# jsourati/nn-active-learning

Hardware: AMD Instinct MI355X
Metric: patches/sec Fisher-scored (32^3, 2-class) (higher is better)
Workload: dtype f32 (fp32 operands split into 16-bit pieces on the 16-bit MFMA, fp32 accumulate: fp16 pairs - 22-23 bits kept per operand, three products - in the conv under the head (forward + backward), in dec1's forward launch and in the other backward launches; bf16 triples - all 24 bits, exact, six products -

## Files before the change

include/alq.h:

```cpp
#ifndef ALQ_H
#define ALQ_H

#include <stddef.h>
#include <stdint.h>

#ifdef __cplusplus
extern "C" {
#endif

typedef struct alq_ctx alq_ctx;
typedef struct alq_model alq_model;

enum { ALQ_OK = 0, ALQ_EINVAL = -1, ALQ_EHIP = -2, ALQ_ENOMEM = -3, ALQ_EUNSUPPORTED = -4 };

enum { ALQ_CONV = 0, ALQ_CONVT = 1, ALQ_POOL = 2, ALQ_FC = 3 };

typedef struct {
    int32_t type;
    int32_t cout;
    int32_t k[3];
    int32_t s[3];
    int32_t relu;
    int32_t skip_src;
} alq_layer_t;
// ... 240 lines not shown
                         int64_t *elems_out);

int alq_debug_set_stamp_buffer(void *d_buf);
int alq_debug_set(int key, int value);
enum {
    ALQ_INFO_SUBNORMALS_OK = 0,
    ALQ_INFO_C3D_FWD = 1,
    ALQ_INFO_C3D_BWD = 2,
    ALQ_INFO_C3D_ONE_ACC = 3,
    ALQ_INFO_FLIP_OVERFLOW = 5,
    ALQ_INFO_F16_DERIVED = 6,
    ALQ_INFO_T3D_FWD = 7,
    ALQ_INFO_T3D_BWD = 8,
    ALQ_INFO_E3D_BWD = 9,
    ALQ_INFO_D3D_FWD = 10,
    ALQ_INFO_D3D_BWD = 11,
    ALQ_INFO_F3D_FWD = 12,
    ALQ_INFO_C3D_BWD_FORM = 13,
    ALQ_INFO_HOST_PACK_ELEMS = 14,
    ALQ_INFO_LSUM = 15,
    ALQ_INFO_DCP_FORM = 16,
    ALQ_INFO_E3D_BWD_FORM = 17,
    ALQ_INFO_C3D_BWD_WAVES = 19,
    ALQ_INFO_C3D_BWD_GRID = 20
};
int alq_model_engine_info(alq_model *m, int what);

int alq_synth_patches(alq_ctx *ctx, uint64_t seed, int64_t first_id, int64_t n,
                      int64_t elems_per_patch, float *d_out);

enum { ALQ_SRC_F32 = 0, ALQ_SRC_F64 = 1, ALQ_SRC_I16 = 2, ALQ_SRC_U8 = 3 };
int alq_vol_pack(alq_ctx *ctx, const void *const *d_src, int m, int src_type, const int32_t *dims, float *d_out);
int alq_mask_pack(alq_ctx *ctx, const uint8_t *d_src, const int32_t *dims, uint8_t *d_out);
int alq_slice_batch_check(const int32_t *h_dims, int nvol, const int32_t *h_desc, int b, const int32_t *crop, int C);
int alq_slice_batch(alq_ctx *ctx, const float *const *h_vols, const uint8_t *const *h_masks, const int32_t *h_dims, int nvol, int m,
                    const int32_t *h_desc, int b, const int32_t *crop, int C, float *d_X, int32_t *d_lab, int64_t *d_counts);
int64_t alq_slice_batch_trip_rows(void);
int alq_slice_batch_launch_samples(void);

#ifdef __cplusplus
}
#endif
#endif
```

nn-active-learning_amd/csrc/alq_internal.h:

```cpp
#pragma once
#include <hip/hip_runtime.h>

#include <cstdint>
#include <cstdio>
#include <memory>
#include <string>
#include <vector>

#include "alq.h"
#include "engine_switches.h"
#include "model_plan.h"

namespace alq {

#define ALQ_HIP(expr)                                                                     \
    do {                                                                                  \
        hipError_t e_ = (expr);                                                           \
        if (e_ != hipSuccess) {                                                           \
            ::alq::set_error("%s:%d: %s -> %s", __FILE__, __LINE__, #expr,               \
                             hipGetErrorString(e_));                                      \
            return ALQ_EHIP;                                                              \
        }                                                                                 \
    } while (0)

// ... 323 lines not shown
void c3d_fwd_pack(C3dPlan *plan, const std::vector<float> &Bmat );
int c3d_fwd_launch(alq_ctx *ctx, const C3dPlan &plan, const View &in, const float *bias, int N, const unsigned *amaxA, const unsigned *amaxB,
                   const float *fc_W, float *fc_part, float *asum_part, unsigned char *fc_bits, float flip_tau);
int c3d_bwd_build(const View &fwd_in, const View &fwd_out, const int k[3], const int lo[3], const int s[3], C3dPlan *plan);
void c3d_bwd_pack(C3dPlan *plan, const std::vector<float> &Bmat_fwd );
void c3d_presplit_vec(const float *v, long long F, int e, std::vector<unsigned short> *out);
int c3d_bwd_launch(alq_ctx *ctx, const C3dPlan &plan, int N, const unsigned char *bits, const void *vec16, int e_in, const unsigned char *maskA,
                   float *dB, float *sumA, float *sumB, int rows_per_wave = 8, int waves_per_simd = 1 ,
                   int *grid_out = nullptr );

struct T3dPlan {
    bool ok = false;
    int kind = 0;
    int w_exp = 0;
    double flops_per_patch = 0;
    std::vector<unsigned short> h_W;
    void *d_W = nullptr;
};
int t3d_build(const View &in, const View &out, const int k[3], const int lo[3], const int s[3], T3dPlan *fwd, T3dPlan *bwd);
void t3d_fwd_pack(T3dPlan *plan, const float *W );
void t3d_bwd_pack(T3dPlan *plan, const float *W);
void t3d8_fwd_pack(T3dPlan *plan, const float *W );
void t3d8_bwd_pack(T3dPlan *plan, const float *W );
int t3d8_bwd_launch(alq_ctx *ctx, const T3dPlan &plan, const View &dout, const View &din, int N, float in_bound, const unsigned char *mask_bits, float *dsum);
int t3d_fwd_launch(alq_ctx *ctx, const T3dPlan &plan, const View &in, const View &out, const float *bias, int N, float *osum, unsigned *out_amax);
int t3d_bwd_launch(alq_ctx *ctx, const T3dPlan &plan, const View &dout, const View &din, int N, float in_bound, const unsigned char *mask_bits,
                   float *dsum);

struct E3dPlan {
    bool ok = false;
    int w_exp = 0;
    double flops_per_patch = 0;
    std::vector<unsigned short> h_Whi, h_Wlo;
    void *d_Whi = nullptr, *d_Wlo = nullptr;
};
int e3d_build(const View &in, const View &out, const int k[3], const int lo[3], const int s[3], E3dPlan *plan);
void e3d_pack(E3dPlan *plan, const float *W );
int e3d_bwd_launch(alq_ctx *ctx, const E3dPlan &plan, int N, const float *skip, const float *dpool, const unsigned char *am2, const unsigned char *sg2,
                   const unsigned char *am1, const unsigned char *sg1, float *dsum2, float *dsum1, float in_bound,
                   bool rows );

struct D3dPlan {
    bool ok = false;
    int w_exp = 0;
    double flops_per_patch = 0;
    std::vector<unsigned short> h_Whi, h_Wlo;
    void *d_Whi = nullptr, *d_Wlo = nullptr;
    std::vector<unsigned short> h_Bhi, h_Blo;
    void *d_Bhi = nullptr, *d_Blo = nullptr;
};
// ... 257 lines not shown
```

nn-active-learning_amd/csrc/engine_switches.h:

```cpp
#ifndef ALQ_ENGINE_SWITCHES_H
#define ALQ_ENGINE_SWITCHES_H
#include <cstddef>
#include <cstdlib>

namespace alq {

enum Knob {
    KNOB_REPEAT = 0,
    KNOB_FLAGS = 1,
    KNOB_NO_BWD_FUSE = 2,
    KNOB_NO_FWD_FUSE = 3,
    KNOB_NO_V3 = 4,
    KNOB_NO_V4 = 5,
    KNOB_NO_POOL_FIRST = 6,
    KNOB_NO_CONV_POOL = 7,
    KNOB_DCP_NARROW = 8,
    KNOB_E3D_GRID_CAP = 9,
    KNOB_C3B7_GRID_CAP = 10,
    ALQ_NKNOBS = 11
};

struct EngineSwitches {
    int knobs[ALQ_NKNOBS] = {0, 0, 0, 0, 0, 0, 0, 0, 0, 0, 0};
    int disable_v2 = 0;
    int disable_v3 = 0;
    int disable_v4 = 0;
    int no_fcgemm = 0;
    int no_split = 0;
    int no_wide2d_rule = 0;
    int no_v3_f16 = 0;
    int no_v3_f16_fwd = 0;
    int no_co_split = 0;
    int no_co_split_f16 = 0;
    int no_class_tiles = 0;
    int no_fc_bits = 0;
    int no_fc_fuse = 0;
    int no_fc_f16 = 0;
    int no_fc_f16_fwd = 0;
    int f16_derived_mask = 0;
    int has_f16_derived_mask = 0;
    int no_f16x2 = 0;
    int no_xcd_order = 0;
    int no_fixed = 0;
    int no_bound16 = 0;
    int no_flipfix = 0;
    int no_presplit = 0;
    int no_signs = 0;
    int no_signs0 = 0;
    int f16_fwd_mask = -1;
    int no_f16_derived = 0;
    int no_light_kernels = 0;
    int no_c3d = 0;
    int c3_bwd_rows = 7;
    int c3_bwd_waves = 2;
    int no_e3d = 0;
    int e3d_rows = 0;
    int no_d3d = 0;
    int no_d3b = 0;
    int no_f3d = 0;
    int no_t3d = 0;
};

enum SwitchRule {
    SW_PRESENT,
    SW_FIRST_IS_1,
    SW_ATOI_EQ,
    SW_INT,
    SW_ROWS
};

struct SwitchRow {
    const char *env;
    size_t member;
    SwitchRule rule;
    int arg;
};

#define ALQ_SW(env, member, rule, arg) {env, offsetof(EngineSwitches, member), rule, arg}
inline const SwitchRow kSwitchTable[] = {
// ... 46 lines not shown
    ALQ_SW("ALQ_NO_T3D", no_t3d, SW_PRESENT, 0),
};
#undef ALQ_SW
inline const int kNumSwitchRows = (int)(sizeof(kSwitchTable) / sizeof(kSwitchTable[0]));

inline int &switch_member(EngineSwitches &sw, const SwitchRow &row) {
    return *reinterpret_cast<int *>(reinterpret_cast<char *>(&sw) + row.member);
}

inline EngineSwitches read_engine_switches() {
    EngineSwitches sw;
    for (const SwitchRow &row : kSwitchTable) {
        const char *v = std::getenv(row.env);
        int &dst = switch_member(sw, row);
        switch (row.rule) {
            case SW_PRESENT:    if (v) dst = 1; break;
            case SW_FIRST_IS_1: if (v && v[0] == '1') dst = 1; break;
            case SW_ATOI_EQ:    if (v && std::atoi(v) == row.arg) dst = 1; break;
            case SW_INT:        if (v) dst = std::atoi(v); break;
            case SW_ROWS:       dst = (v && std::atoi(v) == 4) ? 4 : ((v && std::atoi(v) == 8) ? 8 : 7); break;
        }
    }
    if (const char *v = std::getenv("ALQ_C3D_BWD_WAVES")) sw.c3_bwd_waves = std::atoi(v) == 1 ? 1 : 2;
    return sw;
}

}
#endif
```

nn-active-learning_amd/csrc/igemm2.hip:

```cpp
#include "alq_internal.h"

#include <algorithm>
#include <cmath>
#include <cstring>

namespace alq {

typedef float f32x4 __attribute__((ext_vector_type(4)));
typedef float f32x2 __attribute__((ext_vector_type(2)));

#ifdef ALQ_STAMPS
#define STAMP(var) asm volatile("s_memtime %0\n\ts_waitcnt lgkmcnt(0)" : "=s"(var)::"memory")
#define PHASE_END(idx)                         \
    do {                                       \
        unsigned long long t_now_;             \
        STAMP(t_now_);                         \
        ph[idx] += t_now_ - t_last;            \
        t_last = t_now_;                       \
    } while (0)
#else
#define PHASE_END(idx) do {} while (0)
#endif

constexpr int I2_CBP = 12;
// ... 461 lines not shown
}

void igemm2_pack_weights(Igemm2Plan *p2, const std::vector<float> &Bmat) {
    const Igemm2Args &a = p2->a;
    const int NTW = p2->NTW, Ci = a.Ci, Co = a.Co;
    p2->h_W.assign((size_t)a.nchunks * a.ntaps * NTW * 128, 0.f);
    for (int ch = 0; ch < a.nchunks; ++ch)
        for (int tp = 0; tp < a.ntaps; ++tp)
            for (int nt = 0; nt < NTW; ++nt)
                for (int lane = 0; lane < 64; ++lane)
                    for (int s = 0; s < 2; ++s) {
                        const int c = ch * 8 + 2 * (lane >> 4) + s;
                        const int co = nt * 16 + (lane & 15);
                        if (co < Co)
                            p2->h_W[((((size_t)ch * a.ntaps + tp) * NTW + nt) * 64 + lane) * 2 + s] =
                                Bmat[((size_t)tp * Ci + c) * Co + co];
                    }
}

unsigned long long *g_igemm2_dbg = nullptr;
int g_no_f16x2 = 0;
int g_no_xcd_order = 0;
int g_no_fixed = 0;
int g_dbg_knobs[ALQ_NKNOBS] = {0, 0, 0, 0, 0, 0, 0, 0, 0, 0, 0};

template <int NTW, bool WRES, int GEO, bool SUMS>
static int launch2_s(alq_ctx *ctx, const Igemm2Plan &plan, const Igemm2Args &a, unsigned grid) {
    auto kfn = igemm2_kernel<NTW, WRES, GEO, SUMS>;
    if (plan.lds_bytes > 64 * 1024)
        ALQ_HIP(hipFuncSetAttribute(reinterpret_cast<const void *>(kfn), hipFuncAttributeMaxDynamicSharedMemorySize,
                                    (int)plan.lds_bytes));
    hipLaunchKernelGGL(kfn, dim3(grid), dim3(256), plan.lds_bytes, ctx->stream, a);
    ALQ_HIP(hipGetLastError());
    return ALQ_OK;
}

template <int NTW, bool WRES, int GEO>
static int launch2_t(alq_ctx *ctx, const Igemm2Plan &plan, const Igemm2Args &a, unsigned grid) {
    return (a.osumA || a.osumB) ? launch2_s<NTW, WRES, GEO, true>(ctx, plan, a, grid)
                                : launch2_s<NTW, WRES, GEO, false>(ctx, plan, a, grid);
}

int igemm2_launch(alq_ctx *ctx, const Igemm2Plan &plan, const View &in, const View &out, const float *bias, int relu,
                  int accumulate, int N, int prof_cls, const Igemm2Fuse *fuse) {
    Igemm2Args a = plan.a;
    ALQ_REQUIRE(in.C == a.Ci && in.D == a.ID && in.H == a.IH && in.W == a.IW, ALQ_EINVAL,
                "igemm2: input view does not match plan");
// ... 53 lines not shown
```

nn-active-learning_amd/csrc/model.hip:

```cpp
#include <algorithm>
#include <cstring>
#include <string>

#include "model_types.h"

using namespace alq;

static int g_knob_override[ALQ_NKNOBS] = {-1, -1, -1, -1, -1, -1, -1, -1, -1, -1, -1};

static void apply_knobs(const alq_model *m) {
    for (int k = 0; k < ALQ_NKNOBS; ++k) g_dbg_knobs[k] = g_knob_override[k] >= 0 ? g_knob_override[k] : m->sw.knobs[k];
    g_no_f16x2 = m->sw.no_f16x2;
    g_no_xcd_order = m->sw.no_xcd_order;
    g_no_fixed = m->sw.no_fixed;
}

static int gemm_build(const EngineSwitches &sw, const ConvDesc &d, int max_batch, Gemm *g, const G4Geom *g4 = nullptr) {
    ALQ_TRY(igemm_build_plan(d, max_batch, &g->p1));
    if (g4 && !sw.disable_v4) {
        G4Geom gg = *g4;
        gg.flops_per_patch = g->p1.flops_per_patch;
        ALQ_TRY(igemm4_build_plan(gg, max_batch, &g->p4));
    }
    ALQ_TRY(igemm2_build_plan(g->p1, &g->p2));
    ALQ_TRY(direct_build_plan(g->p1, &g->pd));
    if (sw.disable_v2) { g->p2.ok = false; g->pd.ok = false; }
    ALQ_TRY(igemm3_build_plan(g->p2, &g->p3));
    if (d.ID == 1 && d.IH == 1 && d.IW == 1 && d.tz.size() == 1 && d.sm == 1 && d.so == 1 && !sw.no_fcgemm)
        ALQ_TRY(fcgemm_build_plan(d.Ci, d.Co, &g->pfc));
    if (sw.disable_v3) g->p3.ok = false;
    return ALQ_OK;
// ... 621 lines not shown
            return 0;
        case ALQ_INFO_FLIP_OVERFLOW: {
            ALQ_HIP(hipSetDevice(m->ctx->device));
            if (!m->flip_overflow) return 0;
            unsigned h = 0;
            ALQ_HIP(hipMemcpyAsync(&h, m->flip_overflow, sizeof(unsigned), hipMemcpyDeviceToHost, m->ctx->stream));
            ALQ_HIP(hipStreamSynchronize(m->ctx->stream));
            return h > 0x7fffffffu ? 0x7fffffff : (int)h;
        }
        case ALQ_INFO_F16_DERIVED: return m->last.fwd.f16_derived ? 1 : 0;
        case ALQ_INFO_T3D_FWD: return m->last.fwd.t3f;
        case ALQ_INFO_T3D_BWD: return m->last.bwd.t3b;
        case ALQ_INFO_E3D_BWD: return m->last.bwd.e3b;
        case ALQ_INFO_D3D_FWD: return m->last.fwd.d3f;
        case ALQ_INFO_D3D_BWD: return m->last.bwd.d3b;
        case ALQ_INFO_F3D_FWD: return m->last.fwd.f3f;
        case ALQ_INFO_C3D_BWD_FORM: return m->last.bwd.c3_bwd ? m->sw.c3_bwd_rows : 0;
        case ALQ_INFO_HOST_PACK_ELEMS: return m->host_pack_elems > 0x7fffffffll ? 0x7fffffff : (int)m->host_pack_elems;
        case ALQ_INFO_LSUM: return m->last.lsum;
        case ALQ_INFO_DCP_FORM: return m->last.fwd.dcp;
        case ALQ_INFO_E3D_BWD_FORM: return m->last.bwd.e3b_form;
        case ALQ_INFO_C3D_BWD_WAVES: return m->last.bwd.c3_bwd ? (m->sw.c3_bwd_rows == 7 ? m->sw.c3_bwd_waves : 1) : 0;
        case ALQ_INFO_C3D_BWD_GRID: return m->last.bwd.c3_bwd ? m->last.bwd.c3b_grid : 0;
        default: break;
    }
    set_error("alq_model_engine_info: bad argument");
    return ALQ_EINVAL;
}

int alq_debug_set(int key, int value) {
    ALQ_REQUIRE(key >= 0 && key < ALQ_NKNOBS, ALQ_EINVAL, "alq_debug_set: bad key");
    g_knob_override[key] = value > 0 ? value : -1;
    g_dbg_knobs[key] = value;
    return ALQ_OK;
}

int alq_debug_set_stamp_buffer(void *d_buf) {
    g_igemm2_dbg = reinterpret_cast<unsigned long long *>(d_buf);
    return ALQ_OK;
}

}
```

nn-active-learning_amd/csrc/model_types.h:

```cpp
#pragma once
#include <algorithm>

#include "alq_internal.h"

namespace alq {

struct Layer {
    alq_layer_t spec;
    int pidx = -1;
    View in, out;
    View din, dout;
    int lo[3] = {0, 0, 0};
    bool dense_fc_small = false;
    bool dense_head = false;
    int64_t F = 0;
    int64_t w_elems = 0, b_elems = 0;
    float *d_bias = nullptr;
    float *d_Wp = nullptr;
    std::vector<Gemm> fwd;
    std::vector<Gemm> fwd_co;
    int fwd_co_w = 0;
    Igemm4Plan fwd_all;
    Gemm bwd;
    bool has_bwd = false;
// ... 31 lines not shown
    int hv_src = 0;
    bool hv_stale = false;
    float *hv_W = nullptr;
    double *hv_A = nullptr, *hv_D = nullptr, *hv_Ra = nullptr, *hv_Rd = nullptr;
};

}

struct PassInfo {
    struct Fwd {
        bool head_fused = false;
        bool c3 = false;
        int t3f = 0;
        int d3f = 0;
        int f3f = 0;
        int dcp = 0;
        bool f16_derived = false;
        bool signs_ready[64] = {};
    } fwd;
    struct Bwd {
        bool c3_bwd = false;
        int c3b_grid = 0;
        int t3b = 0;
        int e3b = 0;
        int e3b_form = 0;
        int d3b = 0;
    } bwd;
    int lsum = 0;
    bool call_fisher = false;
};

struct alq_model {
    alq_ctx *ctx = nullptr;
    int max_batch = 0;
    alq::EngineSwitches sw;
    PassInfo last;
    unsigned *amax_a = nullptr, *amax_b = nullptr, *amax_tiles = nullptr;
    unsigned *flip_cnt = nullptr, *flip_list = nullptr;
    int flip_cap = 0;
    unsigned *bound_all = nullptr;
    unsigned *in_amax = nullptr;
    bool v3_fwd_f16 = false;
    unsigned *flip_overflow = nullptr;
    size_t amax_tiles_len = 0;
    int in_dims[4] = {1, 1, 1, 1};
    int nclass = 0;
// ... 94 lines not shown
```

nn-active-learning_amd/csrc/passes.hip:

```cpp
#include <algorithm>
#include <cmath>

#include "model_types.h"

using namespace alq;

static int ensure_bounds(alq_model *m) {
    if (m->bound_all) return ALQ_OK;
    const int nl = (int)m->layers.size();
    ALQ_TRY(m->dalloc(&m->bound_all, (size_t)nl * m->max_batch));
    for (int k = 0; k < nl; ++k) m->layers[k].bound_fwd = m->bound_all + (size_t)k * m->max_batch;
    return ALQ_OK;
}

static int ensure_amax_tiles(alq_model *m, size_t len) {
    if (len <= m->amax_tiles_len) return ALQ_OK;
    ALQ_TRY(m->dalloc(&m->amax_tiles, (size_t)m->max_batch * len));
    m->amax_tiles_len = len;
    return ALQ_OK;
}

static FwdBoundsArgs fwd_bounds_args(const alq_model *m) {
    const int nl = (int)m->layers.size();
    FwdBoundsArgs ba;
// ... 693 lines not shown
}

static int bwd_data_launch(BwdPass &B, BwdStep &s, Igemm2Fuse &fz, const Igemm2Fuse *fuse) {
    alq_model *m = B.m;
    alq_ctx *ctx = m->ctx;
    const int i = s.i, N = B.N, acc = s.acc;
    Layer &ly = m->layers[i];
    Layer *prev = &m->layers[i - 1];
    const bool hand = fuse && bwd_split16_ok(ly) && s.prev_param && !acc && !(B.st[i - 1].dout_bound > 0.f && !m->sw.no_bound16) && prev->pidx > 0 &&
                      prev->bwd.p4.ok && !prev->bwd.p4.multi && prev->bwd.p4.a.PT == 1 && prev->bwd.p4.d_W16 && !prev->dout.split &&
                      ((prev->bwd.p4.NTW == 1 && prev->bwd.p4.fic) || prev->bwd.p4.NTW == 2);
    if (hand) {
        if (!m->amax_a) { ALQ_TRY(m->dalloc(&m->amax_a, (size_t)m->max_batch)); ALQ_TRY(m->dalloc(&m->amax_b, (size_t)m->max_batch)); }
        ALQ_TRY(ensure_amax_tiles(m, (size_t)ly.bwd.p4.a.tpg * 4));
        fz.out_amax = m->amax_tiles;
        fz.amax_from = fz.split > 0 && fz.split < (1 << 29) ? fz.split : 0;
    }
    const unsigned *mine = B.st[i].dout_amax;
    const BwdScale scale = bwd_scale_choice(B, s, fuse != nullptr);
    if (scale != SCALE_NONE && !fuse) { fz = Igemm2Fuse(); fuse = &fz; }
    if (scale == SCALE_MEASURED) fz.in_amax = mine;
    if (scale == SCALE_BOUND) fz.in_bound = B.st[i].dout_bound;
    if (t3d_bwd_applies(m, ly, fuse, acc, hand, s.prev_param)) {
        ALQ_TRY(t3d_bwd_launch(ctx, ly.t3b, ly.dout, ly.din, N, fz.in_bound, fz.mask ? fz.mask_bits : nullptr, fz.osumA));
        s.fused = true;
        m->last.bwd.t3b += 1;
    } else if (d3d_bwd_applies(m, ly, fuse, acc, hand)) {
        ALQ_TRY(d3d_bwd_launch(ctx, ly.d3f, N, ly.dout.p, fz.in_bound, ly.din.p, ly.din.p + ly.din.delta, fz.osumB));
        s.fused = true;
        m->last.bwd.d3b = 1;
    } else {
        ALQ_TRY(gemm_launch(ctx, ly.bwd, ly.dout, ly.din, nullptr, 0, acc, N, PROF_IGEMM_BWD, fuse, &s.fused));
    }
    if (hand) {
        unsigned *dst = mine == m->amax_a ? m->amax_b : m->amax_a;
        ALQ_TRY(k_rowmax_u32(ctx, m->amax_tiles, ly.bwd.p4.a.tpg * 4, N, dst));
        B.st[i - 1].dout_amax = dst;
    }
    return ALQ_OK;
}

static int run_backward_main(alq_model *m, const float *d_x, int N) {
    const int nl = (int)m->layers.size();
    ALQ_REQUIRE(m->nclass == 2, ALQ_EUNSUPPORTED, "Fisher scoring is binary (PW_NNAL.py:766), got %d classes", m->nclass);
    ALQ_TRY(k_fill_unit_cotangent(m->ctx, m->dlogits, N));
    m->last.bwd = {};
    BwdPass B{m, d_x, N};
    B.st.resize(nl);
    bwd_bounds(B);
// ... 34 lines not shown
```

nn-active-learning_amd/csrc/t3d.hip:

```cpp
#include "f16_pair.h"
#include "sweep_common.h"
#ifndef T3_CLOBBER
#define T3_CLOBBER : "memory"
#endif

#include <algorithm>
#include <cmath>
#include <cstdlib>
#include <cstring>
#include <vector>

namespace alq {

struct T3FwdArgs {
    const float *in;
    float *out;
    const unsigned short *W;
    const float *bias;
    float *osum;
    unsigned *out_amax;
    int N;
};
struct T3BwdArgs {
    const float *dout;
// ... 606 lines not shown
        if (N <= 0) return ALQ_OK;
        T8FwdArgs a8;
        a8.in = in.p; a8.out = out.p; a8.W = reinterpret_cast<const unsigned short *>(plan.d_W); a8.bias = bias; a8.osum = osum; a8.N = N;
        ProfScope ps8(ctx, PROF_IGEMM3_FWD, plan.flops_per_patch * N);
        auto go = [&](auto kfn) { return sweep_launch(ctx, kfn, (unsigned)std::min(N, ctx->num_cus), 512, T8_WBYTES + 8 * T8_WAVE, a8); };
        return osum ? go(t3d8_fwd_kernel<true>) : go(t3d8_fwd_kernel<false>);
    }
    ALQ_REQUIRE(in.cs == 16 && in.c0 == 0 && in.split == 0 && out.cs == 8 && out.c0 == 0 && out.split == 0 && in.D == 16 && out.D == 32 && bias,
                ALQ_EINVAL, "t3d: view mismatch");
    SWEEP_REQUIRE_PATCHES(N, "t3d");
    if (N <= 0) return ALQ_OK;
    T3FwdArgs a;
    a.in = in.p; a.out = out.p; a.W = reinterpret_cast<const unsigned short *>(plan.d_W); a.bias = bias; a.osum = osum; a.out_amax = out_amax; a.N = N;
    ProfScope ps(ctx, PROF_IGEMM3_FWD, plan.flops_per_patch * N);
    const dim3 grid(t3_grid(ctx, N));
    if (osum && out_amax) hipLaunchKernelGGL((t3d_fwd_kernel<true, true>), grid, dim3(256), 4 * T3F_WAVE, ctx->stream, a);
    else if (osum) hipLaunchKernelGGL((t3d_fwd_kernel<true, false>), grid, dim3(256), 4 * T3F_WAVE, ctx->stream, a);
    else if (out_amax) hipLaunchKernelGGL((t3d_fwd_kernel<false, true>), grid, dim3(256), 4 * T3F_WAVE, ctx->stream, a);
    else hipLaunchKernelGGL((t3d_fwd_kernel<false, false>), grid, dim3(256), 4 * T3F_WAVE, ctx->stream, a);
    ALQ_HIP(hipGetLastError());
    return ALQ_OK;
}

int t3d_bwd_launch(alq_ctx *ctx, const T3dPlan &plan, const View &dout, const View &din, int N, float in_bound, const unsigned char *mask_bits, float *dsum) {
    ALQ_REQUIRE(plan.ok && plan.d_W, ALQ_EINVAL, "t3d: weights not set");
    if (plan.kind == 8) return t3d8_bwd_launch(ctx, plan, dout, din, N, in_bound, mask_bits, dsum);
    ALQ_REQUIRE(dout.cs == 8 && dout.c0 == 0 && dout.split == 0 && din.cs == 16 && din.c0 == 0 && din.split == 0 && din.D == 16 && dout.D == 32 && in_bound > 0.f,
                ALQ_EINVAL, "t3d: view mismatch");
    SWEEP_REQUIRE_PATCHES(N, "t3d");
    if (N <= 0) return ALQ_OK;
    const int e_in = f16_pair_exp(&in_bound, 1);
    T3BwdArgs a;
    a.dout = dout.p; a.din = din.p; a.W = reinterpret_cast<const unsigned short *>(plan.d_W); a.mask_bits = mask_bits; a.dsum = dsum;
    a.scale = std::ldexp(1.f, e_in); a.inv = std::ldexp(1.f, -(e_in + plan.w_exp)); a.N = N;
    ProfScope ps(ctx, PROF_IGEMM_F16, plan.flops_per_patch * N);
    const dim3 grid(t3_grid(ctx, N));
    if (mask_bits && dsum) hipLaunchKernelGGL((t3d_bwd_kernel<true, true>), grid, dim3(256), 4 * T3B_WAVE, ctx->stream, a);
    else if (mask_bits) hipLaunchKernelGGL((t3d_bwd_kernel<true, false>), grid, dim3(256), 4 * T3B_WAVE, ctx->stream, a);
    else if (dsum) hipLaunchKernelGGL((t3d_bwd_kernel<false, true>), grid, dim3(256), 4 * T3B_WAVE, ctx->stream, a);
    else hipLaunchKernelGGL((t3d_bwd_kernel<false, false>), grid, dim3(256), 4 * T3B_WAVE, ctx->stream, a);
    ALQ_HIP(hipGetLastError());
    return ALQ_OK;
}

}
```

nn-active-learning_amd/csrc/t3d8b.hip:

```cpp
#include "f16_pair.h"
#include "sweep_common.h"

#include <algorithm>
#include <cmath>
#include <cstdlib>
#include <cstring>
#include <vector>

namespace alq {

struct T8BwdArgs {
    const float *dout;
    float *din;
    const unsigned short *W;
    const unsigned char *mask_bits;
    float *dsum;
    float scale, scale11, inv;
    int N;
};

constexpr int T8B_KG = 17 * 16;
constexpr int T8B_PIECE = 2 * T8B_KG;
constexpr int T8B_ROW = 2 * T8B_PIECE + 16;
constexpr int T8B_PLANE = 18 * T8B_ROW + 32;
constexpr int T8B_RING = 3 * T8B_PLANE;
constexpr int T8B_XCH = 4 * 16 * 4;
constexpr int T8B_LDS = T8B_RING + T8B_XCH;

__device__ __host__ inline int t8b_row(int y) { return y * T8B_ROW + ((y >> 1) & 1) * 16; }

__global__ __launch_bounds__(256, 2) void t3d8_bwd_kernel(const T8BwdArgs a) {
    extern __shared__ __attribute__((aligned(16))) char t8lds[];
    const int lane = threadIdx.x & 63, wave = __builtin_amdgcn_readfirstlane((int)(threadIdx.x >> 6));
    const int cb = wave & 1, tp = wave >> 1;
    char *ring = t8lds;
    float *xch = reinterpret_cast<float *>(t8lds + T8B_RING);
    for (int i = threadIdx.x; i < T8B_LDS / 16; i += 256) reinterpret_cast<i32x4 *>(t8lds)[i] = i32x4{0, 0, 0, 0};
    __syncthreads();
    const int n = lane & 15, kg = lane >> 4;
    f16x8 wh[15], wl[15];
#pragma unroll
    for (int c = 0; c < 15; ++c) {
        wh[c] = *reinterpret_cast<const f16x8 *>(a.W + ((size_t)((0 * 2 + cb) * 15 + c) * 64 + lane) * 8);
        wl[c] = *reinterpret_cast<const f16x8 *>(a.W + ((size_t)((1 * 2 + cb) * 15 + c) * 64 + lane) * 8);
    }
#pragma unroll
    for (int c = 0; c < 15; ++c) asm volatile("" : "+v"(wh[c]), "+v"(wl[c]));

    const __amdgpu_buffer_rsrc_t i_rsrc = sw_rsrc(a.dout, (unsigned long long)a.N * 4096 * 64);
    const __amdgpu_buffer_rsrc_t o_rsrc = sw_rsrc(a.din, (unsigned long long)a.N * 512 * 128);
    const __amdgpu_buffer_rsrc_t m_rsrc = sw_rsrc(a.mask_bits, a.mask_bits ? (unsigned long long)a.N * 512 * 8 : 0ull);
    const __amdgpu_buffer_rsrc_t u_rsrc = sw_rsrc(a.dsum, a.dsum ? (unsigned long long)a.N * 512 * 4 : 0ull);

    const int sx = lane >> 2, cq = lane & 3;
    const int w_off = (cq >> 1) * T8B_KG + sx * 16 + (cq & 1) * 8;
    const unsigned ldA = (unsigned)lane * 16u;
    int f01[2][3], f22[2][2];
#pragma unroll
    for (int j = 0; j < 2; ++j) {
        const int qy = 2 * (tp + 2 * j) + (n >> 3), qx = n & 7, h = kg >> 1;
#pragma unroll
        for (int ty = 0; ty < 3; ++ty) f01[j][ty] = t8b_row(2 * qy + ty) + (kg & 1) * T8B_KG + (2 * qx + h) * 16;
        f22[j][0] = t8b_row(2 * qy + h) + (kg & 1) * T8B_KG + (2 * qx + 2) * 16;
        f22[j][1] = t8b_row(2 * qy + 2 + h) + (kg & 1) * T8B_KG + (2 * qx + 2) * 16;
    }
    const unsigned e_out = (unsigned)(cb * 64 + kg * 16), e_msk = (unsigned)(cb * 4 + kg);

    SW_PATCH_ORDER(a.N);

    f32x4 RA[8];
    auto fetch = [&](int p, int pa) __attribute__((always_inline)) {
#pragma unroll
        for (int j = 0; j < 8; ++j) {
            const int k = 8 * wave + j;
            const int pz = pa + (k >> 4);
            const unsigned row = ((unsigned)p * 16u + (unsigned)(pz < 16 ? pz : 15)) * 16u + (unsigned)(k & 15);
            RA[j] = __builtin_bit_cast(f32x4, __builtin_amdgcn_raw_buffer_load_b128(i_rsrc, (int)ldA, sw_s(row * 1024u), 0));
        }
    };
    auto stage = [&](int pa, bool on) __attribute__((always_inline)) {
#pragma unroll
        for (int j = 0; j < 8; ++j) {
            const int k = 8 * wave + j;
            const int pz = pa + (k >> 4), y = k & 15;
            const bool rv = on && pz < 16;
            const float sc = rv ? a.scale : 0.f, sc11 = rv ? a.scale11 : 0.f;
            char *dst = ring + (pz % 3) * T8B_PLANE + t8b_row(y) + w_off;
            const f32x4 g = RA[j];
            const f16x2 h01 = __builtin_convertvector(f32x2{g.x * sc, g.y * sc}, f16x2), h23 = __builtin_convertvector(f32x2{g.z * sc, g.w * sc}, f16x2);
            const f16x2 l01 = __builtin_convertvector(f32x2{__builtin_fmaf((float)h01.x, -2048.f, g.x * sc11), __builtin_fmaf((float)h01.y, -2048.f, g.y * sc11)}, f16x2);
            const f16x2 l23 = __builtin_convertvector(f32x2{__builtin_fmaf((float)h23.x, -2048.f, g.z * sc11), __builtin_fmaf((float)h23.y, -2048.f, g.w * sc11)}, f16x2);
            *reinterpret_cast<i32x2 *>(dst) = i32x2{__builtin_bit_cast(int, h01), __builtin_bit_cast(int, h23)};
            *reinterpret_cast<i32x2 *>(dst + T8B_PIECE) = i32x2{__builtin_bit_cast(int, l01), __builtin_bit_cast(int, l23)};
        }
    };

    const int total = 8 * npw;
    if (total > 0) fetch(patch_of(0), 1);
    for (int g = 0; g < total; ++g) {
        const int i = g >> 3, zq = g & 7;
        const int p = patch_of(i);
        if (zq == 0) {
            f32x4 R0[4];
#pragma unroll
            for (int j = 0; j < 4; ++j)
                R0[j] = __builtin_bit_cast(f32x4, __builtin_amdgcn_raw_buffer_load_b128(i_rsrc, (int)ldA, sw_s((((unsigned)p * 16u) * 16u + (unsigned)(4 * wave + j)) * 1024u), 0));
#pragma unroll
            for (int j = 0; j < 4; ++j) {
                char *dst = ring + t8b_row(4 * wave + j) + w_off;
                const f32x4 gq = R0[j];
                const float sc = a.scale, sc11 = a.scale11;
                const f16x2 h01 = __builtin_convertvector(f32x2{gq.x * sc, gq.y * sc}, f16x2), h23 = __builtin_convertvector(f32x2{gq.z * sc, gq.w * sc}, f16x2);
                const f16x2 l01 = __builtin_convertvector(f32x2{__builtin_fmaf((float)h01.x, -2048.f, gq.x * sc11), __builtin_fmaf((float)h01.y, -2048.f, gq.y * sc11)}, f16x2);
                const f16x2 l23 = __builtin_convertvector(f32x2{__builtin_fmaf((float)h23.x, -2048.f, gq.z * sc11), __builtin_fmaf((float)h23.y, -2048.f, gq.w * sc11)}, f16x2);
                *reinterpret_cast<i32x2 *>(dst) = i32x2{__builtin_bit_cast(int, h01), __builtin_bit_cast(int, h23)};
                *reinterpret_cast<i32x2 *>(dst + T8B_PIECE) = i32x2{__builtin_bit_cast(int, l01), __builtin_bit_cast(int, l23)};
            }
        }
        stage(2 * zq + 1, true);
        unsigned mb[2];
#pragma unroll
        for (int j = 0; j < 2; ++j) {
            const unsigned vox = ((unsigned)p * 8u + (unsigned)zq) * 64u + (unsigned)(tp + 2 * j) * 16u;
            mb[j] = a.mask_bits ? (unsigned)(unsigned char)__builtin_amdgcn_raw_buffer_load_b8(m_rsrc, (int)((unsigned)n * 8u + e_msk), sw_s(vox * 8u), 0) : 0xfu;
        }
        __syncthreads();
        if (g + 1 < total) fetch(patch_of((g + 1) >> 3), 2 * ((g + 1) & 7) + 1);
        f32x4 c[2], cx[2];
#pragma unroll
        for (int j = 0; j < 2; ++j) { c[j] = f32x4{0.f, 0.f, 0.f, 0.f}; cx[j] = f32x4{0.f, 0.f, 0.f, 0.f}; }
#pragma unroll
        for (int tz = 0; tz < 3; ++tz) {
            const char *pl = ring + ((2 * zq + tz) % 3) * T8B_PLANE;
#pragma unroll
            for (int j = 0; j < 2; ++j)
#pragma unroll
                for (int pi = 0; pi < 5; ++pi) {
                    const char *src = pl + (pi < 3 ? f01[j][pi] : f22[j][pi - 3]);
                    const f16x8 xh = *reinterpret_cast<const f16x8 *>(src);
                    const f16x8 xl = *reinterpret_cast<const f16x8 *>(src + T8B_PIECE);
                    cx[j] = __builtin_amdgcn_mfma_f32_16x16x32_f16(wl[tz * 5 + pi], xh, cx[j], 0, 0, 0);
                    c[j] = __builtin_amdgcn_mfma_f32_16x16x32_f16(wh[tz * 5 + pi], xh, c[j], 0, 0, 0);
                    cx[j] = __builtin_amdgcn_mfma_f32_16x16x32_f16(wh[tz * 5 + pi], xl, cx[j], 0, 0, 0);
                }
        }
        float part[2];
#pragma unroll
        for (int j = 0; j < 2; ++j) {
            const unsigned vox = (unsigned)sw_s((((unsigned)p * 8u + (unsigned)zq) * 64u + (unsigned)(tp + 2 * j) * 16u));
            const unsigned m = mb[j];
            const float v0 = (m & 1u) ? __builtin_fmaf(cx[j].x, 0x1p-11f, c[j].x) * a.inv : 0.f, v1 = (m & 2u) ? __builtin_fmaf(cx[j].y, 0x1p-11f, c[j].y) * a.inv : 0.f;
            const float v2 = (m & 4u) ? __builtin_fmaf(cx[j].z, 0x1p-11f, c[j].z) * a.inv : 0.f, v3 = (m & 8u) ? __builtin_fmaf(cx[j].w, 0x1p-11f, c[j].w) * a.inv : 0.f;
            const f32x4 o = f32x4{v0, v1, v2, v3};
            __builtin_amdgcn_raw_buffer_store_b128(__builtin_bit_cast(i32x4, o), o_rsrc, (int)((unsigned)n * 128u + e_out), (int)(vox * 128u), 0);
            float s_ = (v0 + v1) + (v2 + v3);
            s_ += __shfl_xor(s_, 16, 64);
            s_ += __shfl_xor(s_, 32, 64);
            part[j] = s_;
            if (cb == 1 && kg == 0) xch[(tp + 2 * j) * 16 + n] = s_;
            asm volatile("s_nop 3" :: "v"(o) : "memory");
        }
        __syncthreads();
        if (cb == 0 && a.dsum) {
#pragma unroll
            for (int j = 0; j < 2; ++j) {
                const unsigned vox = (unsigned)sw_s((((unsigned)p * 8u + (unsigned)zq) * 64u + (unsigned)(tp + 2 * j) * 16u));
                const float s_ = part[j] + xch[(tp + 2 * j) * 16 + n];
                __builtin_amdgcn_raw_buffer_store_b32(__builtin_bit_cast(int, s_), u_rsrc, (int)(kg == 0 ? (unsigned)n * 4u : SW_OOB), (int)(vox * 4u), 0);
            }
        }
    }
}

void t3d8_bwd_pack(T3dPlan *plan, const float *W) {
    plan->w_exp = f16_pair_exp(W, (size_t)27 * 16 * 32);
    plan->h_W.assign((size_t)2 * 2 * 15 * 64 * 8, 0);
    for (int cb = 0; cb < 2; ++cb)
        for (int tz = 0; tz < 3; ++tz)
            for (int pi = 0; pi < 5; ++pi)
                for (int lane = 0; lane < 64; ++lane) {
                    const int r = lane & 15, kg = lane >> 4, h = kg >> 1;
                    int ty, tx;
                    bool any = true;
                    if (pi < 3) { ty = pi; tx = h; } else if (pi == 3) { ty = h; tx = 2; } else { ty = 2; tx = 2; any = h == 0; }
                    for (int c = 0; c < 8; ++c) {
                        const int co = 8 * (kg & 1) + c, ci = 16 * cb + r;
                        const float w = any ? W[((size_t)((tz * 3 + ty) * 3 + tx) * 16 + co) * 32 + ci] : 0.f;
                        const size_t f = (size_t)(cb * 15 + tz * 5 + pi);
                        f16_pair_split(w, plan->w_exp, 11, &plan->h_W[(((size_t)0 * 30 + f) * 64 + lane) * 8 + c], &plan->h_W[(((size_t)1 * 30 + f) * 64 + lane) * 8 + c]);
                    }
                }
}

int t3d8_bwd_launch(alq_ctx *ctx, const T3dPlan &plan, const View &dout, const View &din, int N, float in_bound, const unsigned char *mask_bits, float *dsum) {
    ALQ_REQUIRE(plan.ok && plan.d_W && plan.kind == 8, ALQ_EINVAL, "t3d8: backward weights not set");
    ALQ_REQUIRE(dout.cs == 16 && dout.c0 == 0 && dout.split == 0 && dout.D == 16 && din.cs == 32 && din.c0 == 0 && din.split == 0 && din.D == 8 && in_bound > 0.f,
                ALQ_EINVAL, "t3d8: view mismatch");
    SWEEP_REQUIRE_PATCHES(N, "t3d8");
    if (N <= 0) return ALQ_OK;
    const int e_in = f16_pair_exp(&in_bound, 1);
    T8BwdArgs a;
    a.dout = dout.p; a.din = din.p; a.W = reinterpret_cast<const unsigned short *>(plan.d_W); a.mask_bits = mask_bits; a.dsum = dsum;
    a.scale = std::ldexp(1.f, e_in); a.scale11 = std::ldexp(1.f, e_in + 11); a.inv = std::ldexp(1.f, -(e_in + plan.w_exp)); a.N = N;
    ProfScope ps(ctx, PROF_IGEMM_F16, plan.flops_per_patch * N);
    return sweep_launch(ctx, t3d8_bwd_kernel, sweep_grid(ctx, N, 2), 256, T8B_LDS, a);
}

}
```

Before: 290,700.

## Prefetch next step's loads before barrier in t3d8 backward kernel

Templates the t3d8 backward kernel on a prefetch flag. When it is on, the plane-0 rows, the mask bytes and the next step's input rows for step g+1 are issued before the barrier, and the mask bytes are double-buffered by step parity, so memory latency overlaps the MFMA work. The loop is unrolled by two for the buffer parity. A grid-cap debug knob and an info query are also added. Prefetch is on by default, at the cost of extra registers and some out-of-bounds dummy loads.

```diff
diff --git a/include/alq.h b/include/alq.h
--- a/include/alq.h
+++ b/include/alq.h
@@ -286,7 +286,8 @@
     ALQ_INFO_DCP_FORM = 16,
     ALQ_INFO_E3D_BWD_FORM = 17,
     ALQ_INFO_C3D_BWD_WAVES = 19,
-    ALQ_INFO_C3D_BWD_GRID = 20
+    ALQ_INFO_C3D_BWD_GRID = 20,
+    ALQ_INFO_T3D8B_PREFETCH = 21
 };
 int alq_model_engine_info(alq_model *m, int what);
 
diff --git a/nn-active-learning_amd/csrc/alq_internal.h b/nn-active-learning_amd/csrc/alq_internal.h
--- a/nn-active-learning_amd/csrc/alq_internal.h
+++ b/nn-active-learning_amd/csrc/alq_internal.h
@@ -369,10 +369,11 @@
 void t3d_bwd_pack(T3dPlan *plan, const float *W);
 void t3d8_fwd_pack(T3dPlan *plan, const float *W );
 void t3d8_bwd_pack(T3dPlan *plan, const float *W );
-int t3d8_bwd_launch(alq_ctx *ctx, const T3dPlan &plan, const View &dout, const View &din, int N, float in_bound, const unsigned char *mask_bits, float *dsum);
+int t3d8_bwd_launch(alq_ctx *ctx, const T3dPlan &plan, const View &dout, const View &din, int N, float in_bound, const unsigned char *mask_bits, float *dsum,
+                    int prefetch );
 int t3d_fwd_launch(alq_ctx *ctx, const T3dPlan &plan, const View &in, const View &out, const float *bias, int N, float *osum, unsigned *out_amax);
 int t3d_bwd_launch(alq_ctx *ctx, const T3dPlan &plan, const View &dout, const View &din, int N, float in_bound, const unsigned char *mask_bits,
-                   float *dsum);
+                   float *dsum, int prefetch8 );
 
 struct E3dPlan {
     bool ok = false;
diff --git a/nn-active-learning_amd/csrc/engine_switches.h b/nn-active-learning_amd/csrc/engine_switches.h
--- a/nn-active-learning_amd/csrc/engine_switches.h
+++ b/nn-active-learning_amd/csrc/engine_switches.h
@@ -17,11 +17,12 @@
     KNOB_DCP_NARROW = 8,
     KNOB_E3D_GRID_CAP = 9,
     KNOB_C3B7_GRID_CAP = 10,
-    ALQ_NKNOBS = 11
+    KNOB_T3D8B_GRID_CAP = 11,
+    ALQ_NKNOBS = 12
 };
 
 struct EngineSwitches {
-    int knobs[ALQ_NKNOBS] = {0, 0, 0, 0, 0, 0, 0, 0, 0, 0, 0};
+    int knobs[ALQ_NKNOBS] = {0, 0, 0, 0, 0, 0, 0, 0, 0, 0, 0, 0};
     int disable_v2 = 0;
     int disable_v3 = 0;
     int disable_v4 = 0;
@@ -55,6 +56,7 @@
     int c3_bwd_waves = 2;
     int no_e3d = 0;
     int e3d_rows = 0;
+    int t3d8b_prefetch = 1;
     int no_d3d = 0;
     int no_d3b = 0;
     int no_f3d = 0;
@@ -147,6 +149,7 @@
         }
     }
     if (const char *v = std::getenv("ALQ_C3D_BWD_WAVES")) sw.c3_bwd_waves = std::atoi(v) == 1 ? 1 : 2;
+    if (const char *v = std::getenv("ALQ_T3D8B_PREFETCH")) sw.t3d8b_prefetch = (v[0] == '0' && std::atoi(v) == 0) ? 0 : 1;
     return sw;
 }
 
diff --git a/nn-active-learning_amd/csrc/igemm2.hip b/nn-active-learning_amd/csrc/igemm2.hip
--- a/nn-active-learning_amd/csrc/igemm2.hip
+++ b/nn-active-learning_amd/csrc/igemm2.hip
@@ -507,7 +507,7 @@
 int g_no_f16x2 = 0;
 int g_no_xcd_order = 0;
 int g_no_fixed = 0;
-int g_dbg_knobs[ALQ_NKNOBS] = {0, 0, 0, 0, 0, 0, 0, 0, 0, 0, 0};
+int g_dbg_knobs[ALQ_NKNOBS] = {0, 0, 0, 0, 0, 0, 0, 0, 0, 0, 0, 0};
 
 template <int NTW, bool WRES, int GEO, bool SUMS>
 static int launch2_s(alq_ctx *ctx, const Igemm2Plan &plan, const Igemm2Args &a, unsigned grid) {
diff --git a/nn-active-learning_amd/csrc/model.hip b/nn-active-learning_amd/csrc/model.hip
--- a/nn-active-learning_amd/csrc/model.hip
+++ b/nn-active-learning_amd/csrc/model.hip
@@ -6,7 +6,7 @@
 
 using namespace alq;
 
-static int g_knob_override[ALQ_NKNOBS] = {-1, -1, -1, -1, -1, -1, -1, -1, -1, -1, -1};
+static int g_knob_override[ALQ_NKNOBS] = {-1, -1, -1, -1, -1, -1, -1, -1, -1, -1, -1, -1};
 
 static void apply_knobs(const alq_model *m) {
     for (int k = 0; k < ALQ_NKNOBS; ++k) g_dbg_knobs[k] = g_knob_override[k] >= 0 ? g_knob_override[k] : m->sw.knobs[k];
@@ -674,6 +674,7 @@
         case ALQ_INFO_E3D_BWD_FORM: return m->last.bwd.e3b_form;
         case ALQ_INFO_C3D_BWD_WAVES: return m->last.bwd.c3_bwd ? (m->sw.c3_bwd_rows == 7 ? m->sw.c3_bwd_waves : 1) : 0;
         case ALQ_INFO_C3D_BWD_GRID: return m->last.bwd.c3_bwd ? m->last.bwd.c3b_grid : 0;
+        case ALQ_INFO_T3D8B_PREFETCH: return m->last.bwd.t3b8 ? 1 + m->sw.t3d8b_prefetch : 0;
         default: break;
     }
     set_error("alq_model_engine_info: bad argument");
diff --git a/nn-active-learning_amd/csrc/model_types.h b/nn-active-learning_amd/csrc/model_types.h
--- a/nn-active-learning_amd/csrc/model_types.h
+++ b/nn-active-learning_amd/csrc/model_types.h
@@ -77,6 +77,7 @@
         bool c3_bwd = false;
         int c3b_grid = 0;
         int t3b = 0;
+        int t3b8 = 0;
         int e3b = 0;
         int e3b_form = 0;
         int d3b = 0;
diff --git a/nn-active-learning_amd/csrc/passes.hip b/nn-active-learning_amd/csrc/passes.hip
--- a/nn-active-learning_amd/csrc/passes.hip
+++ b/nn-active-learning_amd/csrc/passes.hip
@@ -739,9 +739,10 @@
     if (scale == SCALE_MEASURED) fz.in_amax = mine;
     if (scale == SCALE_BOUND) fz.in_bound = B.st[i].dout_bound;
     if (t3d_bwd_applies(m, ly, fuse, acc, hand, s.prev_param)) {
-        ALQ_TRY(t3d_bwd_launch(ctx, ly.t3b, ly.dout, ly.din, N, fz.in_bound, fz.mask ? fz.mask_bits : nullptr, fz.osumA));
+        ALQ_TRY(t3d_bwd_launch(ctx, ly.t3b, ly.dout, ly.din, N, fz.in_bound, fz.mask ? fz.mask_bits : nullptr, fz.osumA, m->sw.t3d8b_prefetch));
         s.fused = true;
         m->last.bwd.t3b += 1;
+        if (ly.t3b.kind == 8) m->last.bwd.t3b8 += 1;
     } else if (d3d_bwd_applies(m, ly, fuse, acc, hand)) {
         ALQ_TRY(d3d_bwd_launch(ctx, ly.d3f, N, ly.dout.p, fz.in_bound, ly.din.p, ly.din.p + ly.din.delta, fz.osumB));
         s.fused = true;
diff --git a/nn-active-learning_amd/csrc/t3d.hip b/nn-active-learning_amd/csrc/t3d.hip
--- a/nn-active-learning_amd/csrc/t3d.hip
+++ b/nn-active-learning_amd/csrc/t3d.hip
@@ -652,9 +652,10 @@
     return ALQ_OK;
 }
 
-int t3d_bwd_launch(alq_ctx *ctx, const T3dPlan &plan, const View &dout, const View &din, int N, float in_bound, const unsigned char *mask_bits, float *dsum) {
+int t3d_bwd_launch(alq_ctx *ctx, const T3dPlan &plan, const View &dout, const View &din, int N, float in_bound, const unsigned char *mask_bits, float *dsum,
+                   int prefetch8) {
     ALQ_REQUIRE(plan.ok && plan.d_W, ALQ_EINVAL, "t3d: weights not set");
-    if (plan.kind == 8) return t3d8_bwd_launch(ctx, plan, dout, din, N, in_bound, mask_bits, dsum);
+    if (plan.kind == 8) return t3d8_bwd_launch(ctx, plan, dout, din, N, in_bound, mask_bits, dsum, prefetch8);
     ALQ_REQUIRE(dout.cs == 8 && dout.c0 == 0 && dout.split == 0 && din.cs == 16 && din.c0 == 0 && din.split == 0 && din.D == 16 && dout.D == 32 && in_bound > 0.f,
                 ALQ_EINVAL, "t3d: view mismatch");
     SWEEP_REQUIRE_PATCHES(N, "t3d");
diff --git a/nn-active-learning_amd/csrc/t3d8b.hip b/nn-active-learning_amd/csrc/t3d8b.hip
--- a/nn-active-learning_amd/csrc/t3d8b.hip
+++ b/nn-active-learning_amd/csrc/t3d8b.hip
@@ -29,6 +29,7 @@
 
 __device__ __host__ inline int t8b_row(int y) { return y * T8B_ROW + ((y >> 1) & 1) * 16; }
 
+template <int PF>
 __global__ __launch_bounds__(256, 2) void t3d8_bwd_kernel(const T8BwdArgs a) {
     extern __shared__ __attribute__((aligned(16))) char t8lds[];
     const int lane = threadIdx.x & 63, wave = __builtin_amdgcn_readfirstlane((int)(threadIdx.x >> 6));
@@ -68,17 +69,18 @@
 
     SW_PATCH_ORDER(a.N);
 
+    constexpr int NM = PF ? 2 : 1;
     f32x4 RA[8];
-    auto fetch = [&](int p, int pa) __attribute__((always_inline)) {
+    auto fetch = [&](int p, int pa, f32x4 *R) __attribute__((always_inline)) {
 #pragma unroll
         for (int j = 0; j < 8; ++j) {
             const int k = 8 * wave + j;
             const int pz = pa + (k >> 4);
             const unsigned row = ((unsigned)p * 16u + (unsigned)(pz < 16 ? pz : 15)) * 16u + (unsigned)(k & 15);
-            RA[j] = __builtin_bit_cast(f32x4, __builtin_amdgcn_raw_buffer_load_b128(i_rsrc, (int)ldA, sw_s(row * 1024u), 0));
-        }
-    };
-    auto stage = [&](int pa, bool on) __attribute__((always_inline)) {
+            R[j] = __builtin_bit_cast(f32x4, __builtin_amdgcn_raw_buffer_load_b128(i_rsrc, (int)ldA, sw_s(row * 1024u), 0));
+        }
+    };
+    auto stage = [&](int pa, bool on, const f32x4 *R) __attribute__((always_inline)) {
 #pragma unroll
         for (int j = 0; j < 8; ++j) {
             const int k = 8 * wave + j;
@@ -86,7 +88,7 @@
             const bool rv = on && pz < 16;
             const float sc = rv ? a.scale : 0.f, sc11 = rv ? a.scale11 : 0.f;
             char *dst = ring + (pz % 3) * T8B_PLANE + t8b_row(y) + w_off;
-            const f32x4 g = RA[j];
+            const f32x4 g = R[j];
             const f16x2 h01 = __builtin_convertvector(f32x2{g.x * sc, g.y * sc}, f16x2), h23 = __builtin_convertvector(f32x2{g.z * sc, g.w * sc}, f16x2);
             const f16x2 l01 = __builtin_convertvector(f32x2{__builtin_fmaf((float)h01.x, -2048.f, g.x * sc11), __builtin_fmaf((float)h01.y, -2048.f, g.y * sc11)}, f16x2);
             const f16x2 l23 = __builtin_convertvector(f32x2{__builtin_fmaf((float)h23.x, -2048.f, g.z * sc11), __builtin_fmaf((float)h23.y, -2048.f, g.w * sc11)}, f16x2);
@@ -94,17 +96,32 @@
             *reinterpret_cast<i32x2 *>(dst + T8B_PIECE) = i32x2{__builtin_bit_cast(int, l01), __builtin_bit_cast(int, l23)};
         }
     };
+    f32x4 R0[4];
+    auto fetch0 = [&](int p, bool on) __attribute__((always_inline)) {
+#pragma unroll
+        for (int j = 0; j < 4; ++j)
+            R0[j] = __builtin_bit_cast(f32x4, __builtin_amdgcn_raw_buffer_load_b128(i_rsrc, (int)(on ? ldA : SW_OOB), sw_s((((unsigned)p * 16u) * 16u + (unsigned)(4 * wave + j)) * 1024u), 0));
+    };
+    unsigned char MB[NM][2];
+    const unsigned nomask = a.mask_bits ? 0u : 0xfu;
+    auto fetchm = [&](int g, unsigned char *mb) __attribute__((always_inline)) {
+        const int p = patch_of(g >> 3), zq = g & 7;
+#pragma unroll
+        for (int j = 0; j < 2; ++j) {
+            const unsigned vox = ((unsigned)p * 8u + (unsigned)zq) * 64u + (unsigned)(tp + 2 * j) * 16u;
+            if (PF == 0 && !a.mask_bits) mb[j] = 0;
+            else mb[j] = (unsigned char)__builtin_amdgcn_raw_buffer_load_b8(m_rsrc, (int)((unsigned)n * 8u + e_msk), sw_s(vox * 8u), 0);
+        }
+    };
 
     const int total = 8 * npw;
-    if (total > 0) fetch(patch_of(0), 1);
-    for (int g = 0; g < total; ++g) {
+    auto step = [&](int g, auto par) __attribute__((always_inline)) {
+        constexpr int b = decltype(par)::value;
+        constexpr int mbi = PF ? b : 0;
         const int i = g >> 3, zq = g & 7;
         const int p = patch_of(i);
         if (zq == 0) {
-            f32x4 R0[4];
-#pragma unroll
-            for (int j = 0; j < 4; ++j)
-                R0[j] = __builtin_bit_cast(f32x4, __builtin_amdgcn_raw_buffer_load_b128(i_rsrc, (int)ldA, sw_s((((unsigned)p * 16u) * 16u + (unsigned)(4 * wave + j)) * 1024u), 0));
+            if constexpr (PF == 0) fetch0(p, true);
 #pragma unroll
             for (int j = 0; j < 4; ++j) {
                 char *dst = ring + t8b_row(4 * wave + j) + w_off;
@@ -117,15 +134,17 @@
                 *reinterpret_cast<i32x2 *>(dst + T8B_PIECE) = i32x2{__builtin_bit_cast(int, l01), __builtin_bit_cast(int, l23)};
             }
         }
-        stage(2 * zq + 1, true);
-        unsigned mb[2];
-#pragma unroll
-        for (int j = 0; j < 2; ++j) {
-            const unsigned vox = ((unsigned)p * 8u + (unsigned)zq) * 64u + (unsigned)(tp + 2 * j) * 16u;
-            mb[j] = a.mask_bits ? (unsigned)(unsigned char)__builtin_amdgcn_raw_buffer_load_b8(m_rsrc, (int)((unsigned)n * 8u + e_msk), sw_s(vox * 8u), 0) : 0xfu;
+        stage(2 * zq + 1, true, RA);
+        if constexpr (PF == 0) fetchm(g, MB[0]);
+        if constexpr (PF >= 1) {
+            fetch0(patch_of(i + 1), zq == 7);
+            fetchm(g + 1, MB[b ^ 1]);
+            fetch(patch_of((g + 1) >> 3), 2 * ((g + 1) & 7) + 1, RA);
         }
         __syncthreads();
-        if (g + 1 < total) fetch(patch_of((g + 1) >> 3), 2 * ((g + 1) & 7) + 1);
+        if constexpr (PF == 0) { if (g + 1 < total) fetch(patch_of((g + 1) >> 3), 2 * ((g + 1) & 7) + 1, RA); }
+        unsigned mb[2] = {(unsigned)MB[mbi][0] | nomask, (unsigned)MB[mbi][1] | nomask};
+        if constexpr (PF >= 1) asm volatile("" : "+v"(mb[0]), "+v"(mb[1]));
         f32x4 c[2], cx[2];
 #pragma unroll
         for (int j = 0; j < 2; ++j) { c[j] = f32x4{0.f, 0.f, 0.f, 0.f}; cx[j] = f32x4{0.f, 0.f, 0.f, 0.f}; }
@@ -161,14 +180,30 @@
             asm volatile("s_nop 3" :: "v"(o) : "memory");
         }
         __syncthreads();
-        if (cb == 0 && a.dsum) {
+        if (PF >= 1 || (cb == 0 && a.dsum)) {
 #pragma unroll
             for (int j = 0; j < 2; ++j) {
                 const unsigned vox = (unsigned)sw_s((((unsigned)p * 8u + (unsigned)zq) * 64u + (unsigned)(tp + 2 * j) * 16u));
                 const float s_ = part[j] + xch[(tp + 2 * j) * 16 + n];
-                __builtin_amdgcn_raw_buffer_store_b32(__builtin_bit_cast(int, s_), u_rsrc, (int)(kg == 0 ? (unsigned)n * 4u : SW_OOB), (int)(vox * 4u), 0);
+                __builtin_amdgcn_raw_buffer_store_b32(__builtin_bit_cast(int, s_), u_rsrc, (int)(cb == 0 && kg == 0 ? (unsigned)n * 4u : SW_OOB), (int)(vox * 4u), 0);
             }
         }
+    };
+    if (total > 0) {
+        if constexpr (PF >= 1) { fetch0(patch_of(0), true); fetchm(0, MB[0]); }
+        fetch(patch_of(0), 1, RA);
+    }
+    int g = 0;
+    if constexpr (PF >= 1) {
+        if (total > 0) {
+            step(0, IC<0>());
+            step(1, IC<1>());
+        }
+        g = 2;
+    }
+    for (; g < total; g += 2) {
+        step(g, IC<0>());
+        step(g + 1, IC<1>());
     }
 }
 
@@ -192,7 +227,7 @@
                 }
 }
 
-int t3d8_bwd_launch(alq_ctx *ctx, const T3dPlan &plan, const View &dout, const View &din, int N, float in_bound, const unsigned char *mask_bits, float *dsum) {
+int t3d8_bwd_launch(alq_ctx *ctx, const T3dPlan &plan, const View &dout, const View &din, int N, float in_bound, const unsigned char *mask_bits, float *dsum, int prefetch) {
     ALQ_REQUIRE(plan.ok && plan.d_W && plan.kind == 8, ALQ_EINVAL, "t3d8: backward weights not set");
     ALQ_REQUIRE(dout.cs == 16 && dout.c0 == 0 && dout.split == 0 && dout.D == 16 && din.cs == 32 && din.c0 == 0 && din.split == 0 && din.D == 8 && in_bound > 0.f,
                 ALQ_EINVAL, "t3d8: view mismatch");
@@ -203,7 +238,10 @@
     a.dout = dout.p; a.din = din.p; a.W = reinterpret_cast<const unsigned short *>(plan.d_W); a.mask_bits = mask_bits; a.dsum = dsum;
     a.scale = std::ldexp(1.f, e_in); a.scale11 = std::ldexp(1.f, e_in + 11); a.inv = std::ldexp(1.f, -(e_in + plan.w_exp)); a.N = N;
     ProfScope ps(ctx, PROF_IGEMM_F16, plan.flops_per_patch * N);
-    return sweep_launch(ctx, t3d8_bwd_kernel, sweep_grid(ctx, N, 2), 256, T8B_LDS, a);
-}
-
-}
+    unsigned g = sweep_grid(ctx, N, 2);
+    if (g_dbg_knobs[KNOB_T3D8B_GRID_CAP] > 0) g = std::min<unsigned>(g, ((unsigned)g_dbg_knobs[KNOB_T3D8B_GRID_CAP] + 7u) / 8u * 8u);
+    if (prefetch == 0) return sweep_launch(ctx, t3d8_bwd_kernel<0>, g, 256, T8B_LDS, a);
+    return sweep_launch(ctx, t3d8_bwd_kernel<1>, g, 256, T8B_LDS, a);
+}
+
+}
```

Result: no change. 291,100 (median of 2 runs) (+0.1%).
